# PKU-VCL-Geometry/GeoSplatting

Hardware: AMD Instinct MI355X
Metric: fwd+bwd views/sec at 2M Gaussians, 800x800 (higher is better)
Workload: dtype f32

## Files before the change

### geosplatting_amd/_lib.py

```python
from __future__ import annotations

import ctypes as C
import os
from typing import Optional

import torch

_HERE = os.path.dirname(os.path.abspath(__file__))
LIB_PATH = os.path.join(_HERE, "libgeosplat_hip.so")

GS_MAX_LEVELS = 16


class GsEnv(C.Structure):
    _fields_ = [("lut", C.c_void_p), ("lut_res", C.c_int), ("base", C.c_void_p), ("base_res", C.c_int),
                ("num_levels", C.c_int), ("levels", C.c_void_p * GS_MAX_LEVELS), ("res", C.c_int * GS_MAX_LEVELS),
                ("min_roughness", C.c_float), ("max_roughness", C.c_float)]


class GsTailView(C.Structure):
    _fields_ = [("viewmat", C.c_void_p), ("K", C.c_void_p), ("cam_pos", C.c_void_p), ("vis_records", C.c_void_p), ("v_packed", C.c_void_p),
                ("packed_index", C.c_void_p), ("W", C.c_int), ("H", C.c_int)]


class GsTileLevel(C.Structure):
    _fields_ = [("R", C.c_int), ("n_mirrors", C.c_int), ("margin", C.c_int), ("bw", C.c_int), ("nb", C.c_int), ("tile_begin", C.c_int),
                ("tile_end", C.c_int), ("reserved", C.c_int), ("src", C.c_void_p), ("scale", C.c_void_p), ("out_scale", C.c_void_p),
                ("bounds", C.c_void_p), ("tiles", C.c_void_p), ("segments", C.c_void_p), ("row_begin", C.c_void_p), ("row_counts", C.c_void_p),
                ("desc", C.c_void_p), ("weights", C.c_void_p), ("dst", C.c_void_p), ("lds_bytes", C.c_size_t)]


class GsDensifyTensor(C.Structure):
    _fields_ = [("src", C.c_void_p), ("dst", C.c_void_p), ("floats_per_row", C.c_int), ("kind", C.c_int)]


class GsTsdfView(C.Structure):
    _fields_ = [("depth_alpha", C.c_void_p), ("viewmat", C.c_void_p), ("K", C.c_void_p), ("W", C.c_int), ("H", C.c_int)]


class GsEnvGrad(C.Structure):
    _fields_ = [("base", C.c_void_p), ("levels", C.c_void_p * GS_MAX_LEVELS)]


SYMBOLS = [
    "gs_last_error", "gs_version", "gs_project_ws_bytes", "gs_project_fwd", "gs_project_fwd_vis", "gs_project_fwd_vis_ex", "gs_isect_emit", "gs_sort_ws_bytes",
    "gs_isect_sort", "gs_isect_bin_ws_bytes", "gs_isect_bin", "gs_isect_offsets", "gs_raster_ws_bytes", "gs_raster_fwd", "gs_raster_prepare", "gs_raster_prepare_vis", "gs_raster_composite", "gs_raster_grad_stride", "gs_raster_bwd", "gs_raster_bwd_acc", "gs_selftest_rcp", "gs_selftest_exp", "gs_selftest_cube_edges", "gs_isect_bin_cap", "gs_isect_offsets_cap", "gs_isect_bin_tiles_cap", "gs_isect_offsets_tiles_cap", "gs_raster_prepare_vis_cap", "gs_raster_composite_cap", "gs_raster_bwd_cap", "gs_raster_bwd_acc_cap", "gs_raster_composite_tone", "gs_raster_bwd_tone_acc", "gs_raster_log_ws_bytes", "gs_raster_composite_tone_log", "gs_raster_bwd_tone_log_acc", "gs_project_bwd_cap", "gs_project_bwd", "gs_project_bwd_ex", "gs_shade_fwd",
    "gs_shade_bwd_ws_bytes", "gs_shade_bwd_plan_blocks", "gs_shade_bwd", "gs_tonemap_fwd", "gs_tonemap_bwd", "gs_tonemap_fwd3", "gs_tonemap_bwd3", "gs_cubemap_mip_fwd", "gs_cubemap_mip_chain_fwd", "gs_cube_sample_linear",
    "gs_cubemap_mip_bwd", "gs_diffuse_cubemap_fwd", "gs_diffuse_cubemap_bwd", "gs_specular_bounds", "gs_specular_bounds_ws_bytes", "gs_specular_bounds_fast", "gs_cube_dir_table",
    "gs_specular_cubemap_fwd", "gs_specular_cubemap_bwd", "gs_specular_tiles_count", "gs_specular_tiles_fill",
    "gs_specular_tiles_check", "gs_specular_tiles_apply", "gs_specular_tiles_apply_multi", "gs_mgadapter_fwd", "gs_mgadapter_bwd", "gs_vertex_normals_fwd",
    "gs_vertex_normals_bwd", "gs_photo_loss_ws_bytes", "gs_photo_loss", "gs_smooth_loss_ws_bytes", "gs_smooth_loss", "gs_hashgrid_fwd", "gs_hashgrid_bwd_ws_bytes", "gs_hashgrid_bwd", "gs_hashgrid_bwd_fixed_ws_bytes", "gs_hashgrid_bwd_fixed", "gs_mlp_wgrad_ws_bytes", "gs_mlp_wgrad",
    "gs_flexicubes_ws_bytes", "gs_flexicubes_count", "gs_flexicubes_fwd", "gs_flexicubes_bwd", "gs_flexicubes_entropy_fwd",
    "gs_flexicubes_entropy_bwd", "gs_front_ws_bytes", "gs_front_fwd", "gs_isect_bin_front_ws_bytes", "gs_isect_bin_front", "gs_isect_bin_front_classes", "gs_tail_bwd", "gs_tail_bwd_multi", "gs_tail_bwd_multi_parts", "gs_tail_priv_ws_bytes", "gs_tail_priv_reduce", "gs_smooth_gather", "gs_smooth_fold", "gs_activation_chain",
    "gs_densify_stats", "gs_densify_ws_bytes", "gs_densify_plan", "gs_densify_fill",
    "gs_surfel_project_ws_bytes", "gs_surfel_project_fwd", "gs_surfel_project_bwd", "gs_surfel_raster_fwd", "gs_surfel_grad_stride",
    "gs_surfel_raster_bwd",
    "gs_tsdf_integrate", "gs_tsdf_extract_ws_bytes", "gs_tsdf_extract_count", "gs_tsdf_extract_fill",
    "gs_meshraster_ws_bytes", "gs_meshraster_fwd", "gs_meshraster_resolve", "gs_meshraster_bwd", "gs_mesh_interp_fwd",
    "gs_mesh_interp_bwd",
    "gs_mesh_topology_bytes", "gs_mesh_topology_build", "gs_meshaa_fwd", "gs_meshaa_bwd",
    "gs_tex2d_fwd", "gs_tex2d_bwd", "gs_meshshade_fwd", "gs_meshshade_bwd",
    "gs_bvh_bytes", "gs_bvh_ws_bytes", "gs_bvh_build", "gs_ray_occluded", "gs_ray_closest",
    "gs_envshade_fwd", "gs_envshade_bwd",
    "gs_denoise_tiled_fits", "gs_denoise_fwd", "gs_denoise_bwd",
]

_lib: Optional[C.CDLL] = None


class GeoSplatHipError(RuntimeError):
    pass


def lib() -> C.CDLL:
    global _lib
    if _lib is None:
        if not os.path.exists(LIB_PATH):
            raise GeoSplatHipError(
                f"{LIB_PATH} not found: build it with `python -m geosplatting_amd.build` "
                "(hipcc --offload-arch=gfx950).  geosplatting_amd has no CPU / PyTorch fallback.")
        l = C.CDLL(LIB_PATH)
        l.gs_last_error.restype = C.c_char_p
        l.gs_project_ws_bytes.restype = C.c_size_t
        l.gs_project_ws_bytes.argtypes = [C.c_int]
        l.gs_sort_ws_bytes.restype = C.c_size_t
        l.gs_sort_ws_bytes.argtypes = [C.c_int64, C.c_int, C.c_int]
# ... 124 lines not shown
```

### geosplatting_amd/csrc/gs_segsort_dev.h

```cpp
#pragma once
#include <stdint.h>

#ifndef GS_SEGSORT_FN
#define GS_SEGSORT_FN __device__ __forceinline__
#endif

typedef unsigned long long gs_u64;

template <bool PAD>
GS_SEGSORT_FN int gs_seg_phys(int i) { return PAD ? i + (i >> 5) : i; }

template <bool F64>
GS_SEGSORT_FN gs_u64 gs_seg_inf() { return F64 ? 0x7ff0000000000000ull : ~0ull; }

template <bool F64>
GS_SEGSORT_FN void gs_seg_cx(gs_u64& a, gs_u64& b)
{
#if defined(__HIP_DEVICE_COMPILE__)
    if (F64) {
        const double x = __builtin_bit_cast(double, a), y = __builtin_bit_cast(double, b);
        double lo, hi;
        asm("v_min_f64 %0, %1, %2" : "=v"(lo) : "v"(x), "v"(y));
        asm("v_max_f64 %0, %1, %2" : "=v"(hi) : "v"(x), "v"(y));
        a = __builtin_bit_cast(gs_u64, lo); b = __builtin_bit_cast(gs_u64, hi);
// ... 60 lines not shown
                if ((r & (1 << s)) == 0) gs_seg_cx<F64>(e[r], e[r | (1 << s)]);
        }
#pragma unroll
        for (int r = 0; r < R; ++r) {
            const int i = (r >= H ? base2 : base) + (r << a);
            if (!GUARD || i < n) buf[gs_seg_phys<PAD>(i)] = e[r];
        }
    }
}

template <int GMAX, bool PAD, bool F64, bool GUARD>
GS_SEGSORT_FN void gs_seg_group_n(int g, gs_u64* buf, int n, int P, int a, bool flip, int tid, int nthreads)
{
    if (g == GMAX) gs_seg_group<GMAX, PAD, F64, GUARD>(buf, n, P, a, flip, tid, nthreads);
    else if constexpr (GMAX > 1) gs_seg_group_n<GMAX - 1, PAD, F64, GUARD>(g, buf, n, P, a, flip, tid, nthreads);
}

#define GS_SEG_SORT_BODY(GMAX, PAD, F64, GUARD, buf, n, P, tid, nthreads, BARRIER)                           \
    do {                                                                                                     \
        gs_seg_first<GMAX, PAD, F64, GUARD>(buf, n, P, tid, nthreads);                                       \
        BARRIER;                                                                                             \
        for (int k_ = 2 << (GMAX), lgk_ = (GMAX) + 1; k_ <= (P); k_ <<= 1, ++lgk_) {                         \
            int rem_ = lgk_;                                                                                 \
            bool flip_ = true;                                                                               \
            while (rem_ > 0) {                                                                               \
                const int g_ = flip_ ? ((rem_ - 1) % (GMAX)) + 1 : (GMAX);                                   \
                gs_seg_group_n<GMAX, PAD, F64, GUARD>(g_, buf, n, P, rem_ - g_, flip_, tid, nthreads);       \
                BARRIER;                                                                                     \
                rem_ -= g_;                                                                                  \
                flip_ = false;                                                                               \
            }                                                                                                \
        }                                                                                                    \
    } while (0)
```

### geosplatting_amd/csrc/gs_sort.hip

```cpp
#include "gs_common.h"
#include "gs_segsort_dev.h"

#include <cstdlib>
#include <cstring>

#define RS_THREADS 256
#define RS_WAVES 4
#define RS_ITEMS 8
#define RS_TILE (RS_THREADS * RS_ITEMS)
#define RS_WCHUNK (64 * RS_ITEMS)

typedef unsigned long long u64;

static int tile_bits(int tile_w, int tile_h)
{
    unsigned n = (unsigned)(tile_w * tile_h);
    int b = 0;
    while (n > 1) { n >>= 1; ++b; }
    return b + 1;
}

struct PairItem { u64 key; int32_t val; };
struct PairIn {
    const u64* keys; const int32_t* vals;
// ... 218 lines not shown
    int32_t* tv = (int32_t*)p;
    const int end_bit = 32 + tile_bits(tile_w, tile_h);
    const int npass = (end_bit + 7) / 8;
    const u64* src_k = (const u64*)isect_ids; const int32_t* src_v = flatten_ids;
    for (int pass = 0; pass < npass; ++pass) {
        const int shift = pass * 8;
        const int nbits = (end_bit - shift) < 8 ? (end_bit - shift) : 8;
        const bool to_out = ((npass - 1 - pass) % 2) == 0;
        u64* dk = to_out ? (u64*)isect_ids_sorted : tk;
        int32_t* dv = to_out ? flatten_ids_sorted : tv;
        const int rc = radix_pass<PairItem>(GsCount{ n_isects, nullptr }, PairIn{ src_k, src_v }, PairDigit{ shift, (1u << nbits) - 1u }, PairOut{ dk, dv }, nbits, table, s);
        if (rc != GS_OK) return rc;
        src_k = dk; src_v = dv;
    }
    return GS_OK;
}

__device__ __forceinline__ void tile_range_sorted(float mx, float my, int radius, int tile_size, int tw, int th,
                                                  int& x0, int& y0, int& x1, int& y1)
{
#pragma clang fp contract(off)
    const float ts = (float)tile_size;
    const float tr = (float)radius / ts;
    const float tx = mx / ts, ty = my / ts;
    const float fx0 = floorf(tx - tr), fy0 = floorf(ty - tr);
    const float fx1 = ceilf(tx + tr), fy1 = ceilf(ty + tr);
    x0 = fx0 < 0.0f ? 0 : (fx0 > (float)tw ? tw : (int)fx0);
    y0 = fy0 < 0.0f ? 0 : (fy0 > (float)th ? th : (int)fy0);
    x1 = fx1 < 0.0f ? 0 : (fx1 > (float)tw ? tw : (int)fx1);
    y1 = fy1 < 0.0f ? 0 : (fy1 > (float)th ? th : (int)fy1);
}

#define EM_THREADS 256
#define EM_PER 4
#define EM_LOOK 4
#define EM_TILE (EM_THREADS * EM_PER)

__global__ void __launch_bounds__(256)
tile_rect_kernel(GsCount vc, const float* __restrict__ means2d, const int32_t* __restrict__ radii, int tile_size, int tile_w, int tile_h,
                 uint2* __restrict__ rect)
{
    const int V = (int)gs_count(vc);
    const int v = blockIdx.x * blockDim.x + threadIdx.x;
    if (v >= V) return;
    const float2 m = *reinterpret_cast<const float2*>(means2d + 2 * (size_t)v);
    int x0 = 0, y0 = 0, x1 = 0, y1 = 0;
    const int r = radii[v];
    if (r > 0) tile_range_sorted(m.x, m.y, r, tile_size, tile_w, tile_h, x0, y0, x1, y1);
    rect[v] = make_uint2((unsigned)x0 | ((unsigned)y0 << 16), (unsigned)x1 | ((unsigned)y1 << 16));
}
__device__ __forceinline__ unsigned rect_count(uint2 q)
{
    const int w = (int)(q.y & 0xffffu) - (int)(q.x & 0xffffu), h = (int)(q.y >> 16) - (int)(q.x >> 16);
    return (w > 0 && h > 0) ? (unsigned)(w * h) : 0u;
}

static size_t bf_state_bytes(int V) { return align256(16 + 2 * (size_t)((V + EM_TILE - 1) / EM_TILE + 1) * sizeof(u64)); }

extern "C" size_t gs_isect_bin_ws_bytes(int V, int64_t n_isects, int tile_w, int tile_h)
{
    (void)tile_w; (void)tile_h;
    const size_t v = V > 0 ? (size_t)V : 1, n = n_isects > 0 ? (size_t)n_isects : 1;
    const size_t tb = table_bytes((int64_t)(v > n ? v : n));
    return tb + 3 * align256(v * 8) + bf_state_bytes((int)v) + 2 * align256(n * 8) + 256;
}

__global__ void capacity_check_kernel(const long long* __restrict__ counts, long long v_cap, long long i_cap, long long* __restrict__ status)
{
// ... 132 lines not shown
                            pv[j] = __hip_atomic_load(&pre[idx], __ATOMIC_RELAXED, __HIP_MEMORY_SCOPE_AGENT);
                            av[j] = __hip_atomic_load(&agg[idx], __ATOMIC_RELAXED, __HIP_MEMORY_SCOPE_AGENT);
                        }
                    }
                    const u64 pmask = __ballot(isP);
                    const int first = pmask ? __builtin_ctzll(pmask) : 64;
                    if (lane <= first) acc += val & ~BF_VALID;
                    if (pmask) done = true;
                }
                pos -= 64 * EM_LOOK;
            }
        }
        const unsigned long long base = gs_wave_sum_u64(acc);
        if (lane == 0) {
            __hip_atomic_store(&pre[block], (u64)(base + total) | BF_VALID, __ATOMIC_RELAXED, __HIP_MEMORY_SCOPE_AGENT);
            s_base = base;
        }
    }
    __syncthreads();
    unsigned long long cur = s_base + before + incl - mine;
#pragma unroll
    for (int k = 0; k < EM_PER; ++k) {
        if (v[k] < 0 || c[k] == 0u) continue;
        const int x0 = (int)(q[k].x & 0xffffu), y0 = (int)(q[k].x >> 16), x1 = (int)(q[k].y & 0xffffu), y1 = (int)(q[k].y >> 16);
        for (int i = y0; i < y1; ++i)
            for (int j = x0; j < x1; ++j) {
                const unsigned t = (unsigned)(i * tile_w + j);
                if (cur < (unsigned long long)item_cap) items[cur] = make_uint2(t, (unsigned)v[k]);
                ++cur;
            }
    }
}

#define SEG_CLASSES 3
#define SEG_CAP0 2048
#define SEG_CAP1 4096
#define SEG_CAP2 16384
#define SEG_GMAX 4
#define SEG_THREADS(cap) ((cap) >> SEG_GMAX > 1024 ? 1024 : ((cap) >> SEG_GMAX))
#define SEG_BINS 64
static size_t seg_lds_bytes(int cap) { return (size_t)(cap + (cap >> 5) + 1) * sizeof(u64); }

extern "C" int gs_isect_bin_front_classes(int* caps, int max)
{
    const int c[SEG_CLASSES] = { SEG_CAP0, SEG_CAP1, SEG_CAP2 };
    for (int i = 0; i < SEG_CLASSES && i < max; ++i) if (caps) caps[i] = c[i];
    return SEG_CLASSES;
}

struct SegLists { unsigned* count; int32_t* lists; };

__device__ __forceinline__ int seg_class(unsigned len) { return len <= SEG_CAP0 ? 0 : (len <= SEG_CAP1 ? 1 : (len <= SEG_CAP2 ? 2 : 3)); }
__device__ __forceinline__ int seg_bin(unsigned len)
{
    const int l2 = 31 - __clz((int)len);
    const int half = l2 > 0 ? (int)((len >> (l2 - 1)) & 1u) : 0;
    return SEG_BINS - 1 - (2 * l2 + half);
}

__global__ void __launch_bounds__(1024)
tile_offsets_scan_kernel(int n_tiles, const unsigned* __restrict__ tile_counts, GsCount nc, int32_t* __restrict__ offsets, SegLists sl)
{
    __shared__ unsigned wsum[16];
    __shared__ unsigned s_bin[(SEG_CLASSES + 1) * SEG_BINS];
    const unsigned n = (unsigned)gs_count(nc);
    const int lane = threadIdx.x & 63, wave = threadIdx.x >> 6;
    if (sl.count && threadIdx.x < (SEG_CLASSES + 1) * SEG_BINS) s_bin[threadIdx.x] = 0u;
    __syncthreads();
    unsigned carry = 0u;
    for (int i0 = 0; i0 < n_tiles; i0 += 1024) {
        const int i = i0 + threadIdx.x;
        const unsigned v = i < n_tiles ? tile_counts[i] : 0u;
        unsigned incl = v;
        incl = gs_wave_incl_scan(incl);
        if (lane == 63) wsum[wave] = incl;
        __syncthreads();
        unsigned before = 0u, all = 0u;
        for (int w = 0; w < 16; ++w) { if (w < wave) before += wsum[w]; all += wsum[w]; }
        if (i < n_tiles) {
            const unsigned o = carry + before + incl - v;
            const unsigned beg = o < n ? o : n, end = o + v < n ? o + v : n;
            offsets[i] = (int32_t)beg;
            if (sl.count && end > beg) atomicAdd(&s_bin[seg_class(end - beg) * SEG_BINS + seg_bin(end - beg)], 1u);
        }
        carry += all;
        __syncthreads();
    }
    if (!sl.count) return;
    if (wave <= SEG_CLASSES) {
        const unsigned v = s_bin[wave * SEG_BINS + lane];
        const unsigned incl = gs_wave_incl_scan(v);
        s_bin[wave * SEG_BINS + lane] = incl - v;
        if (lane == 63) sl.count[wave] = incl;
    }
    __syncthreads();
    for (int i = threadIdx.x; i < n_tiles; i += 1024) {
        const unsigned beg = (unsigned)offsets[i];
        unsigned end = n;
        if (i + 1 < n_tiles) end = (unsigned)__hip_atomic_load(&offsets[i + 1], __ATOMIC_RELAXED, __HIP_MEMORY_SCOPE_WORKGROUP);
        if (end > beg) {
            const int c = seg_class(end - beg);
            const unsigned pos = atomicAdd(&s_bin[c * SEG_BINS + seg_bin(end - beg)], 1u);
            sl.lists[(size_t)c * n_tiles + pos] = i;
        }
    }
}

#define SC_THREADS 512
#define SC_PER 8
#define SC_TILE (SC_THREADS * SC_PER)

__global__ void __launch_bounds__(SC_THREADS)
bin_scatter_kernel(GsCount vc, const unsigned* __restrict__ keys, const uint2* __restrict__ rects, unsigned key_mask, u64 item_bias, int tile_w, int tile_h,
                   const int32_t* __restrict__ offsets, unsigned* __restrict__ cursor, u64* __restrict__ items, unsigned item_cap)
{
    extern __shared__ unsigned s_pos[];
    const int V = (int)gs_count(vc);
    const int n_tiles = tile_w * tile_h;
    const int s0 = (int)blockIdx.x * SC_TILE + (int)threadIdx.x;
    if ((long long)blockIdx.x * SC_TILE >= V) return;
    for (int t = threadIdx.x; t < n_tiles; t += SC_THREADS) s_pos[t] = 0u;
    unsigned key[SC_PER]; uint2 q[SC_PER];
#pragma unroll
    for (int k = 0; k < SC_PER; ++k) {
        const int v = s0 + k * SC_THREADS;
        const int vv = v < V ? v : V - 1;
        key[k] = keys[vv];
        q[k] = rects[vv];
        if (v >= V) q[k] = make_uint2(0u, 0u);
    }
#pragma unroll
    for (int k = 0; k < SC_PER; ++k) {
        int x1 = (int)(q[k].y & 0xffffu), y1 = (int)(q[k].y >> 16);
        x1 = x1 < tile_w ? x1 : tile_w; y1 = y1 < tile_h ? y1 : tile_h;
        q[k].y = (unsigned)x1 | ((unsigned)y1 << 16);
    }
// ... 1 lines not shown
#pragma unroll
    for (int k = 0; k < SC_PER; ++k) {
        const int x0 = (int)(q[k].x & 0xffffu), y0 = (int)(q[k].x >> 16), x1 = (int)(q[k].y & 0xffffu), y1 = (int)(q[k].y >> 16);
        for (int i = y0; i < y1; ++i)
            for (int j = x0; j < x1; ++j) atomicAdd(&s_pos[i * tile_w + j], 1u);
    }
    __syncthreads();
    for (int t0 = threadIdx.x; t0 < n_tiles; t0 += 4 * SC_THREADS) {
        unsigned c[4], o[4], b[4];
#pragma unroll
        for (int u = 0; u < 4; ++u) {
            const int t = t0 + u * SC_THREADS;
            c[u] = t < n_tiles ? s_pos[t] : 0u;
            o[u] = c[u] ? (unsigned)offsets[t] : 0u;
        }
#pragma unroll
        for (int u = 0; u < 4; ++u) b[u] = c[u] ? atomicAdd(&cursor[t0 + u * SC_THREADS], c[u]) : 0u;
#pragma unroll
        for (int u = 0; u < 4; ++u) if (c[u]) s_pos[t0 + u * SC_THREADS] = o[u] + b[u];
    }
    __syncthreads();
#pragma unroll
    for (int k = 0; k < SC_PER; ++k) {
        const int x0 = (int)(q[k].x & 0xffffu), y0 = (int)(q[k].x >> 16), x1 = (int)(q[k].y & 0xffffu), y1 = (int)(q[k].y >> 16);
        const u64 item = item_bias | ((u64)(key[k] & key_mask) << 31) | (u64)(unsigned)(s0 + k * SC_THREADS);
        for (int i = y0; i < y1; ++i)
            for (int j = x0; j < x1; ++j) {
                const unsigned pos = atomicAdd(&s_pos[i * tile_w + j], 1u);
                if (pos < item_cap) items[pos] = item;
            }
    }
}

template <int THREADS, bool GLOBAL, bool F64>
__global__ void __launch_bounds__(THREADS)
seg_sort_kernel(const int32_t* __restrict__ list, const unsigned* __restrict__ list_count, int n_tiles, const int32_t* __restrict__ offsets,
                GsCount ic, GsCount vc, u64* items, int32_t* __restrict__ flat)
{
    extern __shared__ u64 s_seg[];
    if (blockIdx.x >= *list_count) return;
    const int t = list[blockIdx.x];
    const int n_all = (int)gs_count(ic);
    const int beg = offsets[t], end = t + 1 < n_tiles ? offsets[t + 1] : n_all;
    const int n = end - beg;
    if (n <= 0) return;
    const long long V = gs_count(vc);
    const unsigned vmax = V > 0 ? (unsigned)(V - 1) : 0u;
    const int tid = threadIdx.x;
    int P = 1 << SEG_GMAX;
    while (P < n) P <<= 1;
    u64* buf = GLOBAL ? items + beg : s_seg;
    if (!GLOBAL) {
        for (int i = tid; i < P; i += THREADS) s_seg[gs_seg_phys<true>(i)] = i < n ? items[beg + i] : gs_seg_inf<F64>();
        __syncthreads();
    }
    GS_SEG_SORT_BODY(SEG_GMAX, !GLOBAL, F64, GLOBAL, buf, n, P, tid, THREADS, __syncthreads());
    for (int i = tid; i < n; i += THREADS) {
        const unsigned slot = (unsigned)buf[gs_seg_phys<!GLOBAL>(i)] & 0x7fffffffu;
        flat[beg + i] = (int32_t)(slot < vmax ? slot : vmax);
    }
}

__global__ void __launch_bounds__(256)
bin_offsets_tiles_kernel(GsCount nc, const int32_t* __restrict__ tiles, int n_tiles, int32_t* __restrict__ offsets)
{
    const int64_t n = gs_count(nc);
    const int64_t i = (int64_t)blockIdx.x * blockDim.x + threadIdx.x;
    if (n == 0 && i == 0)
        for (int t = 0; t < n_tiles; ++t) offsets[t] = 0;
    if (i >= n) return;
    const int cur = tiles[i];
    if (i == 0) {
        for (int t = 0; t <= cur && t < n_tiles; ++t) offsets[t] = 0;
    } else {
        const int prev = tiles[i - 1];
        for (int t = prev + 1; t <= cur && t < n_tiles; ++t) offsets[t] = (int32_t)i;
    }
    if (i == n - 1)
        for (int t = cur + 1; t < n_tiles; ++t) offsets[t] = (int32_t)n;
}


static size_t tf_state_words(int n_tiles) { return (size_t)n_tiles + SEG_CLASSES + 1; }
static size_t tf_ws_bytes(int64_t n_isects, int n_tiles)
{
    return align256(tf_state_words(n_tiles) * 4) + align256((size_t)(SEG_CLASSES + 1) * n_tiles * 4) + align256((size_t)n_isects * 8) + 256;
}
static size_t bf_radix_ws_bytes(size_t v, size_t n)
{
    return table_bytes((int64_t)(v > n ? v : n)) + 2 * align256(v * 8) + 2 * align256(n * 8) + bf_state_bytes((int)v) + align256(n * 4) + 256;
}

extern "C" size_t gs_isect_bin_front_ws_bytes(int V, int64_t n_isects, int tile_w, int tile_h)
{
    const size_t v = V > 0 ? (size_t)V : 1, n = n_isects > 0 ? (size_t)n_isects : 1;
    const int64_t n_tiles = (int64_t)tile_w * tile_h;
    if (n_tiles > 0 && n_tiles <= BF_HIST_MAX) return tf_ws_bytes((int64_t)n, (int)n_tiles);
    return bf_radix_ws_bytes(v, n);
}

static int bin_front_tile_first(int V, const uint32_t* depth_keys, const uint32_t* tile_rects, const uint32_t* tile_counts,
                                const int64_t* counts_dev, int64_t n_isects, int key_bits, int tile_w, int tile_h, int32_t* flatten_ids_sorted,
                                int32_t* isect_offsets, void* ws, int64_t* status_dev, hipStream_t s)
{
    const int n_tiles = tile_w * tile_h;
    const GsCount vc{ (long long)V, (const long long*)counts_dev }, ic{ (long long)n_isects, counts_dev ? (const long long*)counts_dev + 1 : nullptr };
    char* p = (char*)ws;
    unsigned* cursor = (unsigned*)p;
    unsigned* class_count = cursor + n_tiles; p += align256(tf_state_words(n_tiles) * 4);
    int32_t* lists = (int32_t*)p; p += align256((size_t)(SEG_CLASSES + 1) * n_tiles * 4);
    u64* items = (u64*)p;
    const int n_state_words = (int)tf_state_words(n_tiles);
    hipLaunchKernelGGL(bin_setup_kernel, dim3(gs_cdiv(n_state_words, 256) < 64 ? gs_cdiv(n_state_words, 256) : 64), dim3(256), 0, s, cursor,
                       n_state_words, (const long long*)counts_dev, (long long)V, (long long)n_isects, (long long*)status_dev);
    GS_CHECK_LAUNCH();
    hipLaunchKernelGGL(tile_offsets_scan_kernel, dim3(1), dim3(1024), 0, s, n_tiles, (const unsigned*)tile_counts, ic, isect_offsets,
                       SegLists{ class_count, lists });
    GS_CHECK_LAUNCH();
    const bool f64 = key_bits == 24;
    hipLaunchKernelGGL(bin_scatter_kernel, dim3(gs_cdiv(V, SC_TILE)), dim3(SC_THREADS), (size_t)n_tiles * 4, s, vc,
                       (const unsigned*)depth_keys, (const uint2*)tile_rects, f64 ? 0xffffffu : 0xffffffffu, f64 ? (1ull << 62) : 0ull, tile_w, tile_h,
                       (const int32_t*)isect_offsets, cursor, items, (unsigned)n_isects);
    GS_CHECK_LAUNCH();
    GS_CHECK_HIP(hipFuncSetAttribute((const void*)seg_sort_kernel<SEG_THREADS(SEG_CAP2), false, false>, hipFuncAttributeMaxDynamicSharedMemorySize, (int)seg_lds_bytes(SEG_CAP2)));
    GS_CHECK_HIP(hipFuncSetAttribute((const void*)seg_sort_kernel<SEG_THREADS(SEG_CAP2), false, true>, hipFuncAttributeMaxDynamicSharedMemorySize, (int)seg_lds_bytes(SEG_CAP2)));
    const int caps[SEG_CLASSES + 1] = { 0, SEG_CAP0, SEG_CAP1, SEG_CAP2 };
    for (int c = 0; c <= SEG_CLASSES; ++c) {
        const int64_t most = n_isects / (caps[c] + 1);
        const int grid = (int)(most < n_tiles ? most : n_tiles);
        if (grid == 0) continue;
        const int32_t* list = lists + (size_t)c * n_tiles;
#define SEG_LAUNCH1(T, G, F, LDS) hipLaunchKernelGGL((seg_sort_kernel<T, G, F>), dim3(grid), dim3(T), LDS, s, list, (const unsigned*)(class_count + c), n_tiles, \
                                                     (const int32_t*)isect_offsets, ic, vc, items, flatten_ids_sorted)
#define SEG_LAUNCH(T, G, LDS) do { if (f64) SEG_LAUNCH1(T, G, true, LDS); else SEG_LAUNCH1(T, G, false, LDS); } while (0)
        if (c == 0) SEG_LAUNCH(SEG_THREADS(SEG_CAP0), false, seg_lds_bytes(SEG_CAP0));
        else if (c == 1) SEG_LAUNCH(SEG_THREADS(SEG_CAP1), false, seg_lds_bytes(SEG_CAP1));
        else if (c == 2) SEG_LAUNCH(SEG_THREADS(SEG_CAP2), false, seg_lds_bytes(SEG_CAP2));
        else SEG_LAUNCH(1024, true, 0);
#undef SEG_LAUNCH
#undef SEG_LAUNCH1
        GS_CHECK_LAUNCH();
    }
    return GS_OK;
}

extern "C" int gs_isect_bin_front(int V_cap, const uint32_t* depth_keys, const uint32_t* tile_rects, const uint32_t* tile_counts,
                                  const int64_t* counts_dev, int64_t n_isects_cap, int key_bits, int tile_w, int tile_h, int32_t* flatten_ids_sorted,
                                  int32_t* isect_offsets, void* ws, size_t ws_bytes, int64_t* status_dev, void* stream)
{
    const int V = V_cap;
    const int64_t n_isects = n_isects_cap;
    GS_CHECK_ARG(V >= 0 && n_isects >= 0 && tile_w > 0 && tile_h > 0 && (key_bits == 24 || key_bits == 32), "bad sizes or key width");
    GS_CHECK_ARG(n_isects < (1ll << 31), "n_isects must fit int32");
    GS_CHECK_ARG((int64_t)tile_w * tile_h < (1ll << 24) && tile_w < 65536 && tile_h < 65536, "tile grid too large");
    GS_CHECK_ARG(isect_offsets != nullptr && (counts_dev == nullptr || status_dev != nullptr), "null argument");
    hipStream_t s = (hipStream_t)stream;
    const int n_tiles = tile_w * tile_h;
    if (V == 0 || n_isects == 0) { GS_CHECK_HIP(gs_zero_async(isect_offsets, sizeof(int32_t) * (size_t)n_tiles, s)); return GS_OK; }
    GS_CHECK_ARG(depth_keys != nullptr && tile_rects != nullptr && flatten_ids_sorted != nullptr && ws != nullptr, "null argument");
    if (tile_counts != nullptr && n_tiles <= BF_HIST_MAX) {
        if (ws_bytes < tf_ws_bytes(n_isects, n_tiles)) { gs_set_error("gs_isect_bin_front: workspace too small"); return GS_ENOSPC; }
        return bin_front_tile_first(V, depth_keys, tile_rects, tile_counts, counts_dev, n_isects, key_bits, tile_w, tile_h, flatten_ids_sorted,
                                    isect_offsets, ws, status_dev, s);
    }
    if (ws_bytes < bf_radix_ws_bytes((size_t)V, (size_t)n_isects)) { gs_set_error("gs_isect_bin_front: workspace too small for the radix path (no tile_counts)"); return GS_ENOSPC; }
    const GsCount vc{ (long long)V, (const long long*)counts_dev }, ic{ (long long)n_isects, counts_dev ? (const long long*)counts_dev + 1 : nullptr };
    char* p = (char*)ws;
    unsigned* table = (unsigned*)p; p += table_bytes((int64_t)V > n_isects ? (int64_t)V : n_isects);
    uint2* da = (uint2*)p; p += align256((size_t)V * 8);
    uint2* db = (uint2*)p; p += align256((size_t)V * 8);
    uint2* ia = (uint2*)p; p += align256((size_t)n_isects * 8);
    uint2* ib = (uint2*)p; p += align256((size_t)n_isects * 8);
    unsigned* state = (unsigned*)p; p += bf_state_bytes(V);
    int32_t* tile_ids = (int32_t*)p;
    const int eblocks = (V + EM_TILE - 1) / EM_TILE;
// ... 105 lines not shown
```

### include/geosplat_hip.h

```cpp
#ifndef GEOSPLAT_HIP_H
#define GEOSPLAT_HIP_H

#include <stddef.h>
#include <stdint.h>

#ifdef __cplusplus
extern "C" {
#endif

#define GS_OK            0
#define GS_EINVAL       -1
#define GS_ENOSPC       -2
#define GS_ELAUNCH      -3

#define GS_MAX_LEVELS   16
#define GS_MAX_CHANNELS 32

#define GS_MODE_PBR      0
#define GS_MODE_DIFFUSE  1
#define GS_MODE_SPECULAR 2
#define GS_TONE_NONE     0
#define GS_TONE_NAIVE    1
#define GS_TONE_ACES     2

// ... 251 lines not shown
int gs_hashgrid_bwd_fixed(int N, int L, int F, int log2_T, const float* scalings_host, const float* x, const float* table,
                          const float* v_out, float table_grad_scale, float* v_table, int accumulate, float* v_x, void* ws,
                          size_t ws_bytes, void* stream);

size_t gs_mlp_wgrad_ws_bytes(int64_t N);
int gs_mlp_wgrad(int64_t N, int O, int I, const float* dY, const float* X, float scale, float* dW, int accumulate,
                 void* ws, size_t ws_bytes, void* stream);

size_t gs_flexicubes_ws_bytes(int R0, int R1, int R2);
int gs_flexicubes_count(int R0, int R1, int R2, const float* sdf, void* ws, size_t ws_bytes, int64_t* counts, void* stream);
int gs_flexicubes_fwd(int R0, int R1, int R2, const float* vertices, const float* sdf, const float* alpha,
                      const float* beta, const float* gamma, float weight_scale, float sdf_eps, const void* ws,
                      size_t ws_bytes, int64_t Q, int64_t num_quads, int64_t K, float* out_vertices, int64_t* out_faces,
                      float* L_dev, void* stream);
int gs_flexicubes_bwd(int R0, int R1, int R2, const float* vertices, const float* sdf, const float* alpha,
                      const float* beta, const float* gamma, float weight_scale, float sdf_eps, const void* ws,
                      size_t ws_bytes, int64_t Q, int64_t num_quads, int64_t K, const float* out_vertices,
                      const float* v_out_vertices, const float* v_L_dev, float* g_vd_scratch, float* g_vertices,
                      float* g_sdf, float* g_alpha, float* g_beta, float* g_gamma, void* stream);
int gs_flexicubes_entropy_fwd(int R0, int R1, int R2, const float* sdf, void* ws, size_t ws_bytes, float* out, void* stream);
int gs_flexicubes_entropy_bwd(int R0, int R1, int R2, const float* sdf, const void* ws, size_t ws_bytes, const float* v_out,
                              float* g_sdf, int accumulate, void* stream);

size_t gs_front_ws_bytes(int N);
int gs_front_fwd(int N, const float* means, const float* quats, const float* scales, const float* opacities,
                 const float* normals, const float* kd, const float* ks, const float* viewmat, const float* K,
                 const float* cam_pos, float min_roughness, float max_metallic, int mode, const GsEnv* env,
                 int W, int H, int tile_size, float eps2d, float near_plane, float far_plane, float radius_clip,
                 uint32_t key_base, int key_bits, float* vis_records, uint32_t* depth_keys, uint32_t* tile_rects,
                 uint32_t* tile_counts, int32_t* packed_index ,
                 int tight_tiles, int64_t* counts4, int64_t* status4, void* ws, size_t ws_bytes, void* stream);
size_t gs_isect_bin_front_ws_bytes(int V, int64_t n_isects, int tile_w, int tile_h);
int gs_isect_bin_front_classes(int* caps, int max);
int gs_isect_bin_front(int V_cap, const uint32_t* depth_keys, const uint32_t* tile_rects, const uint32_t* tile_counts,
                       const int64_t* counts_dev, int64_t n_isects_cap, int key_bits, int tile_w, int tile_h, int32_t* flatten_ids_sorted,
                       int32_t* isect_offsets, void* ws, size_t ws_bytes, int64_t* status_dev, void* stream);
int gs_tail_bwd(int V_cap, const int64_t* counts_dev, const float* means, const float* quats, const float* scales,
                const float* opacities, const float* normals, const float* kd, const float* ks, const float* viewmat,
                const float* K, const float* cam_pos, float min_roughness, float max_metallic, int mode, const GsEnv* env,
                int W, int H, float eps2d, const float* vis_records, const float* v_packed, int rec_stride,
                float* v_means, float* v_quats, float* v_scales, float* v_opacities, float* v_normals, float* v_kd, float* v_ks,
                const GsEnvGrad* env_grad, void* priv_ws, size_t priv_ws_bytes, void* stream);
typedef struct GsTailView {
    const float* viewmat; const float* K; const float* cam_pos;
    const float* vis_records; const float* v_packed; const int32_t* packed_index;
    int W, H;
} GsTailView;
int gs_tail_bwd_multi(int N, int n_views, const GsTailView* views , const float* means, const float* quats,
                      const float* scales, const float* opacities, const float* normals, const float* kd, const float* ks,
                      float min_roughness, float max_metallic, int mode, const GsEnv* env, float eps2d, int rec_stride,
                      float* v_means, float* v_quats, float* v_scales, float* v_opacities, float* v_normals, float* v_kd, float* v_ks,
                      int accumulate, const GsEnvGrad* env_grad, void* priv_ws, size_t priv_ws_bytes, void* stream);
int gs_tail_bwd_multi_parts(int parts, int N, int n_views, const GsTailView* views , const float* means, const float* quats,
                            const float* scales, const float* opacities, const float* normals, const float* kd, const float* ks,
                            float min_roughness, float max_metallic, int mode, const GsEnv* env, float eps2d, int rec_stride,
                            float* v_means, float* v_quats, float* v_scales, float* v_opacities, float* v_normals, float* v_kd, float* v_ks,
                            int accumulate, const GsEnvGrad* env_grad, void* priv_ws, size_t priv_ws_bytes, void* stream);
size_t gs_tail_priv_ws_bytes(const GsEnv* env , int mode);
int gs_tail_priv_reduce(const GsEnv* env , int mode, const void* priv_ws, size_t priv_ws_bytes, const GsEnvGrad* env_grad,
                        void* stream);

int gs_smooth_gather(int V_cap, const int64_t* counts_dev, const float* vis_records, const float* kd, const float* ks,
                     const float* normals, float* cols, void* stream);
int gs_smooth_fold(int V_cap, const int64_t* counts_dev, const float* vis_records, const float* v_packed9, int stride9, float* v_packed,
                   int stride, float* v_kd, float* v_ks, float* v_normals, void* stream);

// ... 146 lines not shown
```

Baseline: 750.4.

## Split long tile segments into chunks sorted independently then merged via rank search

Replaces the 16K-capacity segment-sort class with a chunked path: tiles longer than 4096 items are split into 4096-item chunks, each sorted in LDS by its own block, then a rank kernel places each element by binary-searching the other chunks. The goal is to spread very long tile segments across many blocks instead of one large, low-occupancy 1024-thread block. The cost is an extra round trip of items through global memory, an extra kernel launch, and a rank cost that grows with the number of chunks. Tiles above 16 chunks still use the global-memory fallback.

```diff
diff --git a/geosplatting_amd/_lib.py b/geosplatting_amd/_lib.py
--- a/geosplatting_amd/_lib.py
+++ b/geosplatting_amd/_lib.py
@@ -51,7 +51,7 @@
     "gs_specular_tiles_check", "gs_specular_tiles_apply", "gs_specular_tiles_apply_multi", "gs_mgadapter_fwd", "gs_mgadapter_bwd", "gs_vertex_normals_fwd",
     "gs_vertex_normals_bwd", "gs_photo_loss_ws_bytes", "gs_photo_loss", "gs_smooth_loss_ws_bytes", "gs_smooth_loss", "gs_hashgrid_fwd", "gs_hashgrid_bwd_ws_bytes", "gs_hashgrid_bwd", "gs_hashgrid_bwd_fixed_ws_bytes", "gs_hashgrid_bwd_fixed", "gs_mlp_wgrad_ws_bytes", "gs_mlp_wgrad",
     "gs_flexicubes_ws_bytes", "gs_flexicubes_count", "gs_flexicubes_fwd", "gs_flexicubes_bwd", "gs_flexicubes_entropy_fwd",
-    "gs_flexicubes_entropy_bwd", "gs_front_ws_bytes", "gs_front_fwd", "gs_isect_bin_front_ws_bytes", "gs_isect_bin_front", "gs_isect_bin_front_classes", "gs_tail_bwd", "gs_tail_bwd_multi", "gs_tail_bwd_multi_parts", "gs_tail_priv_ws_bytes", "gs_tail_priv_reduce", "gs_smooth_gather", "gs_smooth_fold", "gs_activation_chain",
+    "gs_flexicubes_entropy_bwd", "gs_front_ws_bytes", "gs_front_fwd", "gs_isect_bin_front_ws_bytes", "gs_isect_bin_front", "gs_isect_bin_front_classes", "gs_isect_bin_front_chunking", "gs_tail_bwd", "gs_tail_bwd_multi", "gs_tail_bwd_multi_parts", "gs_tail_priv_ws_bytes", "gs_tail_priv_reduce", "gs_smooth_gather", "gs_smooth_fold", "gs_activation_chain",
     "gs_densify_stats", "gs_densify_ws_bytes", "gs_densify_plan", "gs_densify_fill",
     "gs_surfel_project_ws_bytes", "gs_surfel_project_fwd", "gs_surfel_project_bwd", "gs_surfel_raster_fwd", "gs_surfel_grad_stride",
     "gs_surfel_raster_bwd",
diff --git a/geosplatting_amd/csrc/gs_segsort_dev.h b/geosplatting_amd/csrc/gs_segsort_dev.h
--- a/geosplatting_amd/csrc/gs_segsort_dev.h
+++ b/geosplatting_amd/csrc/gs_segsort_dev.h
@@ -116,3 +116,46 @@
             }                                                                                                \
         }                                                                                                    \
     } while (0)
+
+GS_SEGSORT_FN int gs_seg_chunk_count(int n, int K) { return (int)(((long long)n + K - 1) / K); }
+GS_SEGSORT_FN int gs_seg_chunk_begin(int j, int K) { return j * K; }
+GS_SEGSORT_FN int gs_seg_chunk_len(int n, int j, int K) { const int r = n - j * K; return r < 0 ? 0 : (r < K ? r : K); }
+
+template <int R>
+GS_SEGSORT_FN void gs_seg_lower_bound_n(const gs_u64* a, int n, const gs_u64 (&x)[R], int (&out)[R])
+{
+#pragma unroll
+    for (int r = 0; r < R; ++r) out[r] = 0;
+    int len = n;
+    while (len > 1) {
+        const int half = len >> 1;
+        gs_u64 m[R];
+#pragma unroll
+        for (int r = 0; r < R; ++r) m[r] = a[out[r] + half - 1];
+#pragma unroll
+        for (int r = 0; r < R; ++r) out[r] += m[r] < x[r] ? half : 0;
+        len -= half;
+    }
+    if (len == 1) {
+        gs_u64 m[R];
+#pragma unroll
+        for (int r = 0; r < R; ++r) m[r] = a[out[r]];
+#pragma unroll
+        for (int r = 0; r < R; ++r) out[r] += m[r] < x[r] ? 1 : 0;
+    }
+}
+
+template <int R>
+GS_SEGSORT_FN void gs_seg_rank_n(const gs_u64* seg, int n, int K, int a, const int (&p)[R], const gs_u64 (&x)[R], int (&rank)[R])
+{
+#pragma unroll
+    for (int r = 0; r < R; ++r) rank[r] = p[r];
+    const int c = gs_seg_chunk_count(n, K);
+    for (int b = 0; b < c; ++b) {
+        if (b == a) continue;
+        int lb[R];
+        gs_seg_lower_bound_n<R>(seg + gs_seg_chunk_begin(b, K), gs_seg_chunk_len(n, b, K), x, lb);
+#pragma unroll
+        for (int r = 0; r < R; ++r) rank[r] += lb[r];
+    }
+}
diff --git a/geosplatting_amd/csrc/gs_sort.hip b/geosplatting_amd/csrc/gs_sort.hip
--- a/geosplatting_amd/csrc/gs_sort.hip
+++ b/geosplatting_amd/csrc/gs_sort.hip
@@ -274,8 +274,12 @@
 }
 
 #define EM_THREADS 256
+#ifndef EM_PER
 #define EM_PER 4
+#endif
+#ifndef EM_LOOK
 #define EM_LOOK 4
+#endif
 #define EM_TILE (EM_THREADS * EM_PER)
 
 __global__ void __launch_bounds__(256)
@@ -474,25 +478,42 @@
     }
 }
 
-#define SEG_CLASSES 3
+#define SEG_CLASSES 2
 #define SEG_CAP0 2048
 #define SEG_CAP1 4096
-#define SEG_CAP2 16384
+#define SEG_CHUNK SEG_CAP1
+#define SEG_MAX_CHUNKS 16
 #define SEG_GMAX 4
-#define SEG_THREADS(cap) ((cap) >> SEG_GMAX > 1024 ? 1024 : ((cap) >> SEG_GMAX))
+#define SEG_THREADS(cap) ((cap) >> SEG_GMAX)
 #define SEG_BINS 64
+#define SEG_RANK_THREADS 256
+#define SEG_RANK_PER (SEG_CHUNK / SEG_RANK_THREADS)
+#ifndef SEG_GENERAL_THREADS
+#define SEG_GENERAL_THREADS 1024
+#endif
 static size_t seg_lds_bytes(int cap) { return (size_t)(cap + (cap >> 5) + 1) * sizeof(u64); }
 
 extern "C" int gs_isect_bin_front_classes(int* caps, int max)
 {
-    const int c[SEG_CLASSES] = { SEG_CAP0, SEG_CAP1, SEG_CAP2 };
+    const int c[SEG_CLASSES] = { SEG_CAP0, SEG_CAP1 };
     for (int i = 0; i < SEG_CLASSES && i < max; ++i) if (caps) caps[i] = c[i];
     return SEG_CLASSES;
 }
 
-struct SegLists { unsigned* count; int32_t* lists; };
-
-__device__ __forceinline__ int seg_class(unsigned len) { return len <= SEG_CAP0 ? 0 : (len <= SEG_CAP1 ? 1 : (len <= SEG_CAP2 ? 2 : 3)); }
+extern "C" void gs_isect_bin_front_chunking(int* chunk_items, int* max_chunks)
+{
+    if (chunk_items) *chunk_items = SEG_CHUNK;
+    if (max_chunks) *max_chunks = SEG_MAX_CHUNKS;
+}
+
+#define SEG_KINDS 4
+struct SegLists { unsigned* count; int32_t* list0; int32_t* list1; int32_t* listg; };
+static int64_t seg_chunk_entries_max(int64_t n_isects) { return n_isects / SEG_CHUNK + n_isects / (SEG_CHUNK + 1); }
+
+__device__ __forceinline__ int seg_kind(unsigned len)
+{
+    return len <= SEG_CAP0 ? 0 : (len <= SEG_CAP1 ? 1 : (len <= (unsigned)SEG_CHUNK * SEG_MAX_CHUNKS ? 2 : 3));
+}
 __device__ __forceinline__ int seg_bin(unsigned len)
 {
     const int l2 = 31 - __clz((int)len);
@@ -504,10 +525,11 @@
 tile_offsets_scan_kernel(int n_tiles, const unsigned* __restrict__ tile_counts, GsCount nc, int32_t* __restrict__ offsets, SegLists sl)
 {
     __shared__ unsigned wsum[16];
-    __shared__ unsigned s_bin[(SEG_CLASSES + 1) * SEG_BINS];
+    __shared__ unsigned s_bin[SEG_KINDS * SEG_BINS];
+    __shared__ unsigned s_total[SEG_KINDS];
     const unsigned n = (unsigned)gs_count(nc);
     const int lane = threadIdx.x & 63, wave = threadIdx.x >> 6;
-    if (sl.count && threadIdx.x < (SEG_CLASSES + 1) * SEG_BINS) s_bin[threadIdx.x] = 0u;
+    if (sl.count && threadIdx.x < SEG_KINDS * SEG_BINS) s_bin[threadIdx.x] = 0u;
     __syncthreads();
     unsigned carry = 0u;
     for (int i0 = 0; i0 < n_tiles; i0 += 1024) {
@@ -523,27 +545,41 @@
             const unsigned o = carry + before + incl - v;
             const unsigned beg = o < n ? o : n, end = o + v < n ? o + v : n;
             offsets[i] = (int32_t)beg;
-            if (sl.count && end > beg) atomicAdd(&s_bin[seg_class(end - beg) * SEG_BINS + seg_bin(end - beg)], 1u);
+            if (sl.count && end > beg) {
+                const int kind = seg_kind(end - beg);
+                if (kind == 2) atomicAdd(&s_bin[2 * SEG_BINS], (unsigned)gs_seg_chunk_count((int)(end - beg), SEG_CHUNK));
+                else atomicAdd(&s_bin[kind * SEG_BINS + seg_bin(end - beg)], 1u);
+            }
         }
         carry += all;
         __syncthreads();
     }
     if (!sl.count) return;
-    if (wave <= SEG_CLASSES) {
+    if (wave < SEG_KINDS) {
         const unsigned v = s_bin[wave * SEG_BINS + lane];
         const unsigned incl = gs_wave_incl_scan(v);
         s_bin[wave * SEG_BINS + lane] = incl - v;
-        if (lane == 63) sl.count[wave] = incl;
-    }
-    __syncthreads();
+        if (lane == 63) s_total[wave] = incl;
+    }
+    __syncthreads();
+    const unsigned n_chunks = s_total[2];
+    if (threadIdx.x == 0) { sl.count[0] = s_total[0]; sl.count[1] = n_chunks + s_total[1]; sl.count[2] = n_chunks; sl.count[3] = s_total[3]; }
     for (int i = threadIdx.x; i < n_tiles; i += 1024) {
         const unsigned beg = (unsigned)offsets[i];
         unsigned end = n;
         if (i + 1 < n_tiles) end = (unsigned)__hip_atomic_load(&offsets[i + 1], __ATOMIC_RELAXED, __HIP_MEMORY_SCOPE_WORKGROUP);
         if (end > beg) {
-            const int c = seg_class(end - beg);
-            const unsigned pos = atomicAdd(&s_bin[c * SEG_BINS + seg_bin(end - beg)], 1u);
-            sl.lists[(size_t)c * n_tiles + pos] = i;
+            const int kind = seg_kind(end - beg);
+            if (kind == 2) {
+                const int c = gs_seg_chunk_count((int)(end - beg), SEG_CHUNK);
+                const unsigned pos = atomicAdd(&s_bin[2 * SEG_BINS], (unsigned)c);
+                for (int j = 0; j < c; ++j) sl.list1[pos + j] = i | (j << 24);
+            } else {
+                const unsigned pos = atomicAdd(&s_bin[kind * SEG_BINS + seg_bin(end - beg)], 1u);
+                if (kind == 0) sl.list0[pos] = i;
+                else if (kind == 1) sl.list1[n_chunks + pos] = i;
+                else sl.listg[pos] = i;
+            }
         }
     }
 }
@@ -611,18 +647,27 @@
     }
 }
 
-template <int THREADS, bool GLOBAL, bool F64>
+template <int THREADS, bool GLOBAL, bool F64, bool CHUNKS>
 __global__ void __launch_bounds__(THREADS)
 seg_sort_kernel(const int32_t* __restrict__ list, const unsigned* __restrict__ list_count, int n_tiles, const int32_t* __restrict__ offsets,
                 GsCount ic, GsCount vc, u64* items, int32_t* __restrict__ flat)
 {
     extern __shared__ u64 s_seg[];
     if (blockIdx.x >= *list_count) return;
-    const int t = list[blockIdx.x];
+    const int entry = list[blockIdx.x];
+    const int t = CHUNKS ? (entry & 0xffffff) : entry;
     const int n_all = (int)gs_count(ic);
-    const int beg = offsets[t], end = t + 1 < n_tiles ? offsets[t + 1] : n_all;
-    const int n = end - beg;
+    int beg = offsets[t];
+    const int end = t + 1 < n_tiles ? offsets[t + 1] : n_all;
+    int n = end - beg;
     if (n <= 0) return;
+    const bool chunk = CHUNKS && n > SEG_CHUNK;
+    if (chunk) {
+        const int j = (int)((unsigned)entry >> 24);
+        beg += gs_seg_chunk_begin(j, SEG_CHUNK);
+        n = gs_seg_chunk_len(n, j, SEG_CHUNK);
+        if (n <= 0) return;
+    }
     const long long V = gs_count(vc);
     const unsigned vmax = V > 0 ? (unsigned)(V - 1) : 0u;
     const int tid = threadIdx.x;
@@ -634,9 +679,44 @@
         __syncthreads();
     }
     GS_SEG_SORT_BODY(SEG_GMAX, !GLOBAL, F64, GLOBAL, buf, n, P, tid, THREADS, __syncthreads());
+    if (chunk) {
+        for (int i = tid; i < n; i += THREADS) items[beg + i] = buf[gs_seg_phys<!GLOBAL>(i)];
+        return;
+    }
     for (int i = tid; i < n; i += THREADS) {
         const unsigned slot = (unsigned)buf[gs_seg_phys<!GLOBAL>(i)] & 0x7fffffffu;
         flat[beg + i] = (int32_t)(slot < vmax ? slot : vmax);
+    }
+}
+
+__global__ void __launch_bounds__(SEG_RANK_THREADS)
+seg_rank_kernel(const int32_t* __restrict__ list, const unsigned* __restrict__ list_count, int n_tiles, const int32_t* __restrict__ offsets,
+                GsCount ic, GsCount vc, const u64* __restrict__ items, int32_t* __restrict__ flat)
+{
+    if (blockIdx.x >= *list_count) return;
+    const int entry = list[blockIdx.x];
+    const int t = entry & 0xffffff, j = (int)((unsigned)entry >> 24);
+    const int n_all = (int)gs_count(ic);
+    const int beg = offsets[t], end = t + 1 < n_tiles ? offsets[t + 1] : n_all;
+    const int n = end - beg;
+    const int cn = gs_seg_chunk_len(n, j, SEG_CHUNK);
+    if (n <= SEG_CHUNK || cn <= 0) return;
+    const long long V = gs_count(vc);
+    const unsigned vmax = V > 0 ? (unsigned)(V - 1) : 0u;
+    const u64* seg = items + beg;
+    const u64* mine = seg + gs_seg_chunk_begin(j, SEG_CHUNK);
+    int p[SEG_RANK_PER], rank[SEG_RANK_PER]; u64 x[SEG_RANK_PER];
+#pragma unroll
+    for (int k = 0; k < SEG_RANK_PER; ++k) {
+        p[k] = (int)threadIdx.x + k * SEG_RANK_THREADS;
+        x[k] = mine[p[k] < cn ? p[k] : cn - 1];
+    }
+    gs_seg_rank_n<SEG_RANK_PER>(seg, n, SEG_CHUNK, j, p, x, rank);
+#pragma unroll
+    for (int k = 0; k < SEG_RANK_PER; ++k) {
+        if (p[k] >= cn) continue;
+        const unsigned slot = (unsigned)x[k] & 0x7fffffffu;
+        flat[beg + rank[k]] = (int32_t)(slot < vmax ? slot : vmax);
     }
 }
 
@@ -660,10 +740,12 @@
 }
 
 
-static size_t tf_state_words(int n_tiles) { return (size_t)n_tiles + SEG_CLASSES + 1; }
+static size_t tf_state_words(int n_tiles) { return (size_t)n_tiles + SEG_KINDS; }
+static size_t tf_list1_entries(int64_t n_isects, int n_tiles) { return (size_t)n_tiles + (size_t)seg_chunk_entries_max(n_isects); }
+static size_t tf_list_words(int64_t n_isects, int n_tiles) { return 2 * (size_t)n_tiles + tf_list1_entries(n_isects, n_tiles); }
 static size_t tf_ws_bytes(int64_t n_isects, int n_tiles)
 {
-    return align256(tf_state_words(n_tiles) * 4) + align256((size_t)(SEG_CLASSES + 1) * n_tiles * 4) + align256((size_t)n_isects * 8) + 256;
+    return align256(tf_state_words(n_tiles) * 4) + align256(tf_list_words(n_isects, n_tiles) * 4) + align256((size_t)n_isects * 8) + 256;
 }
 static size_t bf_radix_ws_bytes(size_t v, size_t n)
 {
@@ -686,40 +768,42 @@
     const GsCount vc{ (long long)V, (const long long*)counts_dev }, ic{ (long long)n_isects, counts_dev ? (const long long*)counts_dev + 1 : nullptr };
     char* p = (char*)ws;
     unsigned* cursor = (unsigned*)p;
-    unsigned* class_count = cursor + n_tiles; p += align256(tf_state_words(n_tiles) * 4);
-    int32_t* lists = (int32_t*)p; p += align256((size_t)(SEG_CLASSES + 1) * n_tiles * 4);
+    unsigned* list_count = cursor + n_tiles; p += align256(tf_state_words(n_tiles) * 4);
+    int32_t* list0 = (int32_t*)p;
+    int32_t* list1 = list0 + n_tiles;
+    int32_t* listg = list1 + tf_list1_entries(n_isects, n_tiles);
+    p += align256(tf_list_words(n_isects, n_tiles) * 4);
     u64* items = (u64*)p;
     const int n_state_words = (int)tf_state_words(n_tiles);
     hipLaunchKernelGGL(bin_setup_kernel, dim3(gs_cdiv(n_state_words, 256) < 64 ? gs_cdiv(n_state_words, 256) : 64), dim3(256), 0, s, cursor,
                        n_state_words, (const long long*)counts_dev, (long long)V, (long long)n_isects, (long long*)status_dev);
     GS_CHECK_LAUNCH();
     hipLaunchKernelGGL(tile_offsets_scan_kernel, dim3(1), dim3(1024), 0, s, n_tiles, (const unsigned*)tile_counts, ic, isect_offsets,
-                       SegLists{ class_count, lists });
+                       SegLists{ list_count, list0, list1, listg });
     GS_CHECK_LAUNCH();
     const bool f64 = key_bits == 24;
     hipLaunchKernelGGL(bin_scatter_kernel, dim3(gs_cdiv(V, SC_TILE)), dim3(SC_THREADS), (size_t)n_tiles * 4, s, vc,
                        (const unsigned*)depth_keys, (const uint2*)tile_rects, f64 ? 0xffffffu : 0xffffffffu, f64 ? (1ull << 62) : 0ull, tile_w, tile_h,
                        (const int32_t*)isect_offsets, cursor, items, (unsigned)n_isects);
     GS_CHECK_LAUNCH();
-    GS_CHECK_HIP(hipFuncSetAttribute((const void*)seg_sort_kernel<SEG_THREADS(SEG_CAP2), false, false>, hipFuncAttributeMaxDynamicSharedMemorySize, (int)seg_lds_bytes(SEG_CAP2)));
-    GS_CHECK_HIP(hipFuncSetAttribute((const void*)seg_sort_kernel<SEG_THREADS(SEG_CAP2), false, true>, hipFuncAttributeMaxDynamicSharedMemorySize, (int)seg_lds_bytes(SEG_CAP2)));
-    const int caps[SEG_CLASSES + 1] = { 0, SEG_CAP0, SEG_CAP1, SEG_CAP2 };
-    for (int c = 0; c <= SEG_CLASSES; ++c) {
-        const int64_t most = n_isects / (caps[c] + 1);
-        const int grid = (int)(most < n_tiles ? most : n_tiles);
-        if (grid == 0) continue;
-        const int32_t* list = lists + (size_t)c * n_tiles;
-#define SEG_LAUNCH1(T, G, F, LDS) hipLaunchKernelGGL((seg_sort_kernel<T, G, F>), dim3(grid), dim3(T), LDS, s, list, (const unsigned*)(class_count + c), n_tiles, \
-                                                     (const int32_t*)isect_offsets, ic, vc, items, flatten_ids_sorted)
-#define SEG_LAUNCH(T, G, LDS) do { if (f64) SEG_LAUNCH1(T, G, true, LDS); else SEG_LAUNCH1(T, G, false, LDS); } while (0)
-        if (c == 0) SEG_LAUNCH(SEG_THREADS(SEG_CAP0), false, seg_lds_bytes(SEG_CAP0));
-        else if (c == 1) SEG_LAUNCH(SEG_THREADS(SEG_CAP1), false, seg_lds_bytes(SEG_CAP1));
-        else if (c == 2) SEG_LAUNCH(SEG_THREADS(SEG_CAP2), false, seg_lds_bytes(SEG_CAP2));
-        else SEG_LAUNCH(1024, true, 0);
+    const auto tiles_longer_than = [&](int64_t len) { const int64_t most = n_isects / (len + 1); return (int)(most < n_tiles ? most : n_tiles); };
+    const int n_chunks_max = (int)seg_chunk_entries_max(n_isects);
+    const int grid0 = tiles_longer_than(0), grid1 = tiles_longer_than(SEG_CAP0) + n_chunks_max;
+    const int gridg = tiles_longer_than((int64_t)SEG_CHUNK * SEG_MAX_CHUNKS);
+#define SEG_LAUNCH1(T, G, F, CH, LDS, grid, list, count) hipLaunchKernelGGL((seg_sort_kernel<T, G, F, CH>), dim3(grid), dim3(T), LDS, s, (const int32_t*)(list), \
+                                                     (const unsigned*)(count), n_tiles, (const int32_t*)isect_offsets, ic, vc, items, flatten_ids_sorted)
+#define SEG_LAUNCH(T, G, CH, LDS, grid, list, count) do { if (grid > 0) { if (f64) SEG_LAUNCH1(T, G, true, CH, LDS, grid, list, count); \
+                                                          else SEG_LAUNCH1(T, G, false, CH, LDS, grid, list, count); GS_CHECK_LAUNCH(); } } while (0)
+    SEG_LAUNCH(SEG_THREADS(SEG_CAP0), false, false, seg_lds_bytes(SEG_CAP0), grid0, list0, list_count + 0);
+    SEG_LAUNCH(SEG_THREADS(SEG_CAP1), false, true, seg_lds_bytes(SEG_CAP1), grid1, list1, list_count + 1);
+    if (n_chunks_max > 0) {
+        hipLaunchKernelGGL(seg_rank_kernel, dim3(n_chunks_max), dim3(SEG_RANK_THREADS), 0, s, (const int32_t*)list1, (const unsigned*)(list_count + 2),
+                           n_tiles, (const int32_t*)isect_offsets, ic, vc, (const u64*)items, flatten_ids_sorted);
+        GS_CHECK_LAUNCH();
+    }
+    SEG_LAUNCH(SEG_GENERAL_THREADS, true, false, 0, gridg, listg, list_count + 3);
 #undef SEG_LAUNCH
 #undef SEG_LAUNCH1
-        GS_CHECK_LAUNCH();
-    }
     return GS_OK;
 }
 
diff --git a/include/geosplat_hip.h b/include/geosplat_hip.h
--- a/include/geosplat_hip.h
+++ b/include/geosplat_hip.h
@@ -307,6 +307,7 @@
                  int tight_tiles, int64_t* counts4, int64_t* status4, void* ws, size_t ws_bytes, void* stream);
 size_t gs_isect_bin_front_ws_bytes(int V, int64_t n_isects, int tile_w, int tile_h);
 int gs_isect_bin_front_classes(int* caps, int max);
+void gs_isect_bin_front_chunking(int* chunk_items, int* max_chunks);
 int gs_isect_bin_front(int V_cap, const uint32_t* depth_keys, const uint32_t* tile_rects, const uint32_t* tile_counts,
                        const int64_t* counts_dev, int64_t n_isects_cap, int key_bits, int tile_w, int tile_h, int32_t* flatten_ids_sorted,
                        int32_t* isect_offsets, void* ws, size_t ws_bytes, int64_t* status_dev, void* stream);
```

Result: no change. 755.8, median of 6 (+0.7%).
